# strukturag/libheif

Measured on NVIDIA H100. Metric: megapixels/sec HEIC-grid decode->RGB, higher is better.
Workload: dtype u8

## Files before the change

libheif_b200/csrc/b200_hevc_recon.cu:

```cuda
#include "b200_hevc.h"

namespace b200 {

#ifndef B200_RECON_MIN_BLOCKS
#define B200_RECON_MIN_BLOCKS 5
#endif
constexpr int WARPS = 4;
constexpr int PAD = 16;
constexpr int MT32_OFF = 0, MT16_OFF = 32 * 36, MT8_OFF = MT16_OFF + 16 * 20;
constexpr int MAT_BYTES = MT8_OFF + 8 * 12;
constexpr int REF_STRIDE = 136;

struct WarpLayout { int tile, top, res, tmp, desc, total; };
__host__ __device__ inline WarpLayout warp_layout(int log2ctb, int bps) {
  const int ctb = 1 << log2ctb, tb = ctb < 32 ? ctb : 32;
  WarpLayout L; int o = 0;
  L.tile = o; o += ctb * (ctb + PAD) * bps;
  L.top = o; o += (2 * PAD + 2 * ctb + 32) * bps;
  o = (o + 15) & ~15;
  L.res = o; o += ctb * ctb * 2;
  L.tmp = o; o += (tb * (tb + 2) * 2 > 1024 ? tb * (tb + 2) * 2 : 1024);
  L.desc = o; o += (ctb / 4) * (ctb / 4) * 8;
  L.total = (o + 15) & ~15;
  return L;
}

__constant__ int8_t c_dct[32] = {64, 90, 90, 90, 89, 88, 87, 85, 83, 82, 80, 78, 75, 73, 70, 67,
                                 64, 61, 57, 54, 50, 46, 43, 38, 36, 31, 25, 22, 18, 13, 9, 4};
__constant__ int8_t c_angle[35] = {0, 0, 32, 26, 21, 17, 13, 9, 5, 2, 0, -2, -5, -9, -13, -17, -21, -26, -32,
                                   -26, -21, -17, -13, -9, -5, -2, 0, 2, 5, 9, 13, 17, 21, 26, 32};
__constant__ int16_t c_inv_angle[35] = {0, 0, 0, 0, 0, 0, 0, 0, 0, 0, 0, -4096, -1638, -910, -630, -482, -390, -315, -256,
                                        -315, -390, -482, -630, -910, -1638, -4096, 0, 0, 0, 0, 0, 0, 0, 0, 0};
__constant__ uint8_t c_qpc[14] = {29, 30, 31, 32, 33, 33, 34, 34, 35, 35, 36, 36, 37, 37};
__constant__ uint8_t c_level_scale[6] = {40, 45, 51, 57, 64, 72};

__device__ __forceinline__ int clip3i(int lo, int hi, int v) { return min(max(v, lo), hi); }
__device__ __forceinline__ unsigned morton4(unsigned x, unsigned y) {
  unsigned sx = (x & 1) | ((x & 2) << 1) | ((x & 4) << 2) | ((x & 8) << 3);
  unsigned sy = (y & 1) | ((y & 2) << 1) | ((y & 4) << 2) | ((y & 8) << 3);
  return sx | (sy << 1);
}
__device__ __forceinline__ unsigned ld_acquire(const unsigned* p) {
  unsigned v; asm volatile("ld.relaxed.gpu.global.u32 %0, [%1];" : "=r"(v) : "l"(p) : "memory"); return v;
}
__device__ __forceinline__ void st_release(unsigned* p, unsigned v) {
  asm volatile("st.release.gpu.global.u32 [%0], %1;" ::"l"(p), "r"(v) : "memory");
}
__device__ __forceinline__ void bulk_store(void* g, const void* s, unsigned bytes) {
  asm volatile("cp.async.bulk.global.shared::cta.bulk_group [%0], [%1], %2;" ::"l"(g), "r"((unsigned)__cvta_generic_to_shared(s)), "r"(bytes) : "memory");
}

template <bool LIVE, class T> __device__ __forceinline__ T ld_cmd(const T* p) { return LIVE ? __ldcg(p) : *p; }
template <bool LIVE> __device__ __forceinline__ TuCmd ld_tu(const TuCmd* p) { const uint4 v = ld_cmd<LIVE>(reinterpret_cast<const uint4*>(p)); return TuCmd{v.x, v.y, v.z, v.w}; }
template <bool LIVE> __device__ __forceinline__ CoefEntry ld_coef(const CoefEntry* p) { const unsigned v = ld_cmd<LIVE>(reinterpret_cast<const unsigned*>(p)); CoefEntry e; e.pos = (uint16_t)(v & 0xffff); e.level = (int16_t)(v >> 16); return e; }
template <bool LIVE> __device__ __forceinline__ CtuInfo ld_ctu(const CtuInfo* p) {
  CtuInfo c; const uint2* s = reinterpret_cast<const uint2*>(p); uint2* d = reinterpret_cast<uint2*>(&c);
#pragma unroll
  for (int i = 0; i < (int)(sizeof(CtuInfo) / 8); i++) d[i] = ld_cmd<LIVE>(s + i);
  return c;
}

__device__ __forceinline__ int chroma_qp(int qpy, int off, int bd, int cfmt = 1) {
  const int qbd = 6 * (bd - 8);
  const int qpi = clip3i(-qbd, 57, qpy + off);
  const int qpc = cfmt != 1 ? min(qpi, 51) : (qpi < 30 ? qpi : (qpi >= 43 ? qpi - 6 : c_qpc[qpi - 30]));
  return qpc + qbd;
}

__device__ __forceinline__ int dequant(int level, int qp, int bd_shift, int m) {
  const long long scale = (long long)(c_level_scale[qp % 6] << (qp / 6)) * m;
  const long long t = ((long long)level * scale + (1LL << (bd_shift - 1))) >> bd_shift;
  return (int)(t < -32768 ? -32768 : (t > 32767 ? 32767 : t));
}

__device__ __forceinline__ unsigned make_desc(int bx, int by, int lg, int mode, int coded0, int coded1, int tw, int th, int shx, int cx0, int cy0, int cw, int ch,
                                              bool nbL, bool nbAL, bool nbA, bool nbAR) {
  const int n = 1 << lg;
  const bool fL = bx > 0 || nbL, fT = by > 0 || nbA;
  const bool fC = (bx > 0 && by > 0) ? true : (bx > 0 ? nbA : (by > 0 ? nbL : nbAL));
  const unsigned me = morton4((unsigned)(bx << shx) >> 2, (unsigned)by >> 2);
  bool tr = false, bl = false;
  if (cx0 + bx + n < cw) {
    if (by > 0) { if (bx + n < tw) tr = morton4((unsigned)((bx + n) << shx) >> 2, (unsigned)(by - 1) >> 2) < me; }
    else tr = (bx + n < tw) ? nbA : nbAR;
  }
  if (cy0 + by + n < ch && by + n < th) {
    if (bx > 0) bl = morton4((unsigned)((bx - 1) << shx) >> 2, (unsigned)(by + n) >> 2) < me; else bl = nbL;
  }
  const int trc = tr ? min(n, cw - (cx0 + bx + n)) : 0, blc = bl ? min(n, ch - (cy0 + by + n)) : 0;
  return (unsigned)(bx >> 2) | ((unsigned)(by >> 2) << 4) | ((unsigned)(lg - 2) << 8) | ((unsigned)mode << 10) | ((unsigned)coded0 << 16) | ((unsigned)coded1 << 17) |
         ((unsigned)fL << 18) | ((unsigned)fC << 19) | ((unsigned)fT << 20) | ((unsigned)(blc >> 2) << 21) | ((unsigned)(trc >> 2) << 25);
}

template <bool LIVE>
__device__ __forceinline__ void residual4_lane(int16_t* scr, int lane, const CoefEntry* __restrict__ ce, int nnz, int qp, int bd, bool dst, bool tskip, bool raw, int16_t* out,
                                               const uint8_t* __restrict__ sf) {
  int16_t* my = scr + lane;
#pragma unroll
  for (int p = 0; p < 16; p++) my[p * 32] = 0;
  const int bd_shift = bd - 3;
#pragma unroll 1
  for (int i = 0; i < nnz; i++) {
    const CoefEntry e = ld_coef<LIVE>(&ce[i]);
    my[(e.pos & 15) * 32] = raw ? e.level : (int16_t)dequant(e.level, qp, bd_shift, sf ? (int)__ldg(sf + (e.pos & 15)) : 16);
  }
  int c[16];
#pragma unroll
  for (int p = 0; p < 16; p++) c[p] = my[p * 32];
  const int bs2 = 20 - bd, rnd = 1 << (bs2 - 1);
  unsigned* o32 = reinterpret_cast<unsigned*>(out);
  if (raw) {
#pragma unroll
    for (int p = 0; p < 16; p += 2) o32[p >> 1] = (unsigned)(c[p] & 0xffff) | ((unsigned)c[p + 1] << 16);
    return;
  }
  if (tskip) {
#pragma unroll
    for (int p = 0; p < 16; p += 2) {
      const int r0 = ((c[p] << 7) + rnd) >> bs2, r1 = ((c[p + 1] << 7) + rnd) >> bs2;
      o32[p >> 1] = (unsigned)(r0 & 0xffff) | ((unsigned)r1 << 16);
    }
    return;
  }
  int t[16];
#pragma unroll
  for (int x = 0; x < 4; x++) {
    const int c0 = c[x], c1 = c[4 + x], c2 = c[8 + x], c3 = c[12 + x];
    int e0, e1, e2, e3;
    if (dst) {
      e0 = 29 * c0 + 74 * c1 + 84 * c2 + 55 * c3; e1 = 55 * c0 + 74 * c1 - 29 * c2 - 84 * c3;
      e2 = 74 * c0 - 74 * c2 + 74 * c3;           e3 = 84 * c0 - 74 * c1 + 55 * c2 - 29 * c3;
    } else {
      const int a = 64 * (c0 + c2), b = 64 * (c0 - c2), o0 = 83 * c1 + 36 * c3, o1 = 36 * c1 - 83 * c3;
      e0 = a + o0; e1 = b + o1; e2 = b - o1; e3 = a - o0;
    }
    t[x * 4 + 0] = clip3i(-32768, 32767, (e0 + 64) >> 7); t[x * 4 + 1] = clip3i(-32768, 32767, (e1 + 64) >> 7);
    t[x * 4 + 2] = clip3i(-32768, 32767, (e2 + 64) >> 7); t[x * 4 + 3] = clip3i(-32768, 32767, (e3 + 64) >> 7);
  }
#pragma unroll
  for (int y = 0; y < 4; y++) {
    const int c0 = t[y], c1 = t[4 + y], c2 = t[8 + y], c3 = t[12 + y];
    int e0, e1, e2, e3;
    if (dst) {
      e0 = 29 * c0 + 74 * c1 + 84 * c2 + 55 * c3; e1 = 55 * c0 + 74 * c1 - 29 * c2 - 84 * c3;
      e2 = 74 * c0 - 74 * c2 + 74 * c3;           e3 = 84 * c0 - 74 * c1 + 55 * c2 - 29 * c3;
    } else {
      const int a = 64 * (c0 + c2), b = 64 * (c0 - c2), o0 = 83 * c1 + 36 * c3, o1 = 36 * c1 - 83 * c3;
      e0 = a + o0; e1 = b + o1; e2 = b - o1; e3 = a - o0;
    }
    const int r0 = (e0 + rnd) >> bs2, r1 = (e1 + rnd) >> bs2, r2 = (e2 + rnd) >> bs2, r3 = (e3 + rnd) >> bs2;
    o32[y * 2] = (unsigned)(r0 & 0xffff) | ((unsigned)r1 << 16);
    o32[y * 2 + 1] = (unsigned)(r2 & 0xffff) | ((unsigned)r3 << 16);
  }
}

template <bool LIVE>
__device__ __noinline__ void residual_big(int16_t* rs, int16_t* tmp, const int8_t* __restrict__ mat, const CoefEntry* __restrict__ ce, int nnz, int lg, int qp, int bd, int lane,
                                          const uint8_t* __restrict__ sf, int sf_dc, bool raw) {
  const int n = 1 << lg;
  unsigned* z = reinterpret_cast<unsigned*>(rs);
#pragma unroll 1
  for (int i = lane; i < n * n / 2; i += 32) z[i] = 0;
  __syncwarp();
  const int bd_shift = bd + lg - 5;
  int maxrow = 0, maxcol = 0;
#pragma unroll 1
  for (int i = lane; i < nnz; i += 32) {
    const CoefEntry e = ld_coef<LIVE>(&ce[i]);
    const int pos = e.pos & (n * n - 1);
    const int x = pos & (n - 1), y = pos >> lg;
    int m = 16;
    if (sf) m = (pos == 0 && lg >= 4) ? sf_dc : (int)__ldg(sf + ((y >> (lg - 3)) << 3) + (x >> (lg - 3)));
    rs[raw ? pos : x * n + y] = raw ? e.level : (int16_t)dequant(e.level, qp, bd_shift, m);
    maxrow = max(maxrow, y); maxcol = max(maxcol, x);
  }
  maxrow = __reduce_max_sync(0xffffffffu, maxrow); maxcol = __reduce_max_sync(0xffffffffu, maxcol);
  __syncwarp();
  if (raw) return;
  const int8_t* mt = mat + (lg == 5 ? MT32_OFF : (lg == 4 ? MT16_OFF : MT8_OFF));
  const int ms = n + 4, P2 = n + 2;
  const int kq1 = (maxrow >> 2) + 1, ncol = ((maxcol >> 2) + 1) << 2;
#pragma unroll 1
  for (int i = lane; i < n * ncol; i += 32) {
    const int y = i & (n - 1), x = i >> lg;
    const int2* c = reinterpret_cast<const int2*>(rs + x * n);
    const int* mq = reinterpret_cast<const int*>(mt + y * ms);
    int e = 0;
#pragma unroll 2
    for (int q = 0; q < kq1; q++) { const int2 a = c[q]; const int bq = mq[q]; e = __dp2a_lo(a.x, bq, e); e = __dp2a_hi(a.y, bq, e); }
    tmp[y * P2 + x] = (int16_t)clip3i(-32768, 32767, (e + 64) >> 7);
  }
  __syncwarp();
  const int bs2 = 20 - bd, rnd = 1 << (bs2 - 1), kq2 = ncol >> 2;
#pragma unroll 1
  for (int p = lane; p < n * n; p += 32) {
    const int x = p & (n - 1), y = p >> lg;
    const int* u = reinterpret_cast<const int*>(tmp + y * P2);
    const int* mq = reinterpret_cast<const int*>(mt + x * ms);
    int e = 0;
#pragma unroll 2
    for (int q = 0; q < kq2; q++) { const int bq = mq[q]; e = __dp2a_lo(u[2 * q], bq, e); e = __dp2a_hi(u[2 * q + 1], bq, e); }
    rs[p] = (int16_t)((e + rnd) >> bs2);
  }
  __syncwarp();
}

template <typename P>
__device__ __forceinline__ void predict_tb(const uint2 d, P* tl, const P* tp, const int16_t* rs, int16_t* rf, int S, int l, int lpc, unsigned gmask, int cidx, bool luma, bool smooth, int bd, int strong_en) {
  const int bx = (int)(d.x & 15) << 2, by = (int)((d.x >> 4) & 15) << 2, lg = 2 + (int)((d.x >> 8) & 3), mode = (int)((d.x >> 10) & 63);
  const int n = 1 << lg, n2 = 2 * n, n4 = 4 * n;
  const bool coded = (d.x >> (16 + cidx)) & 1, pcm = (d.x >> 29) & 1;
  const bool fL = (d.x >> 18) & 1, fC = (d.x >> 19) & 1, fT = (d.x >> 20) & 1;
  const int blc = (int)((d.x >> 21) & 15) << 2, trc = (int)((d.x >> 25) & 15) << 2;
  const int first = blc ? n - blc : (fL ? n : (fC ? n2 : (fT ? n2 + 1 : (trc ? 3 * n + 1 : -1))));
  const P* colL = tl + by * S + PAD + bx - 1;
  const P* rowA = (by > 0 ? tl + (by - 1) * S : tp) + PAD + bx;
  int dcs = 0;
  const bool small = n4 < lpc;
  const int jn = small ? n4 + 1 : n4;
#pragma unroll 1
  for (int j = l; j < jn; j += lpc) {
    const int i = j == n4 ? n2 : (j < n2 ? j : j + 1);
    int v = 1 << (bd - 1);
    if (first >= 0) {
      int s = first;
      if (blc && i >= n - blc) s = min(i, n - 1);
      if (fL && i >= n) s = min(i, n2 - 1);
      if (fC && i >= n2) s = n2;
      if (fT && i > n2) s = min(i, 3 * n);
      if (trc && i > 3 * n) s = min(i, 3 * n + trc);
      v = s < n2 ? (int)colL[(n2 - 1 - s) * S] : (int)rowA[s - n2 - 1];
    }
    rf[i] = (int16_t)v;
    if ((i >= n && i < n2) || (i > n2 && i <= 3 * n)) dcs += v;
  }
  if (!small && l == 0) {
    int v = 1 << (bd - 1);
    if (first >= 0) {
      int s = first;
      if (blc) s = n - 1;
      if (fL) s = n2 - 1;
      if (fC) s = n2;
      v = s < n2 ? (int)colL[(n2 - 1 - s) * S] : (int)rowA[s - n2 - 1];
    }
    rf[n2] = (int16_t)v;
  }
  __syncwarp();
  const int16_t* ref = rf;
  if (smooth && mode != 1 && n != 4) {
    const int dist = min(abs(mode - 26), abs(mode - 10));
    const int thr = n == 8 ? 7 : (n == 16 ? 1 : 0);
    if (dist > thr) {
      const int corner = rf[n2], bl = rf[0], tr = rf[n4];
      const bool strong = strong_en && n == 32 && abs(corner + tr - 2 * rf[3 * n]) < (1 << (bd - 5)) && abs(corner + bl - 2 * rf[n]) < (1 << (bd - 5));
      int16_t* rb = rf + REF_STRIDE;
#pragma unroll 1
      for (int i = l; i <= n4; i += lpc) {
        int v;
        if (i == 0 || i == n4) v = rf[i];
        else if (strong) {
          if (i == n2) v = corner;
          else if (i < n2) { const int y = n2 - 1 - i; v = ((63 - y) * corner + (y + 1) * bl + 32) >> 6; }
          else { const int x = i - n2 - 1; v = ((63 - x) * corner + (x + 1) * tr + 32) >> 6; }
        } else v = (rf[i - 1] + 2 * rf[i] + rf[i + 1] + 2) >> 2;
        rb[i] = (int16_t)v;
      }
      __syncwarp();
      ref = rb;
    }
  }
  const int maxv = (1 << bd) - 1;
#define LEFT(y) ((int)ref[n2 - 1 - (y)])
#define TOP(x) ((int)ref[n2 + 1 + (x)])
  int dc = 0;
  if (mode == 1) dc = (__reduce_add_sync(gmask, dcs) + n) >> (lg + 1);
  const int ang = c_angle[mode], ia = c_inv_angle[mode];
  const bool edge = luma && n < 32;
  const int16_t* rsb = rs + d.y;
  P* out = tl + by * S + PAD + bx;
#pragma unroll 1
  for (int e = l; e < n * n; e += lpc) {
    const int x = e & (n - 1), y = e >> lg;
    int v;
    if (pcm) { out[y * S + x] = (P)rsb[e]; continue; }
    if (mode == 0) v = ((n - 1 - x) * LEFT(y) + (x + 1) * TOP(n) + (n - 1 - y) * TOP(x) + (y + 1) * LEFT(n) + n) >> (lg + 1);
    else if (mode == 1) {
      v = dc;
      if (edge) {
        if (x == 0 && y == 0) v = (LEFT(0) + 2 * dc + TOP(0) + 2) >> 2;
        else if (y == 0) v = (TOP(x) + 3 * dc + 2) >> 2;
        else if (x == 0) v = (LEFT(y) + 3 * dc + 2) >> 2;
      }
    } else if (mode >= 18) {
      const int idx = ((y + 1) * ang) >> 5, f = ((y + 1) * ang) & 31;
      const int k0 = x + idx + 1, k1 = k0 + 1;
      const int a = k0 >= 0 ? TOP(k0 - 1) : LEFT(-1 + ((k0 * ia + 128) >> 8));
      if (f) { const int b = k1 >= 0 ? TOP(k1 - 1) : LEFT(-1 + ((k1 * ia + 128) >> 8)); v = ((32 - f) * a + f * b + 16) >> 5; } else v = a;
      if (mode == 26 && edge && x == 0) v = clip3i(0, maxv, TOP(0) + ((LEFT(y) - LEFT(-1)) >> 1));
    } else {
      const int idx = ((x + 1) * ang) >> 5, f = ((x + 1) * ang) & 31;
      const int k0 = y + idx + 1, k1 = k0 + 1;
      const int a = k0 >= 0 ? LEFT(k0 - 1) : TOP(-1 + ((k0 * ia + 128) >> 8));
      if (f) { const int b = k1 >= 0 ? LEFT(k1 - 1) : TOP(-1 + ((k1 * ia + 128) >> 8)); v = ((32 - f) * a + f * b + 16) >> 5; } else v = a;
      if (mode == 10 && edge && y == 0) v = clip3i(0, maxv, LEFT(0) + ((TOP(x) - TOP(-1)) >> 1));
    }
    if (coded) v = clip3i(0, maxv, v + (int)rsb[e]);
    out[y * S + x] = (P)v;
  }
#undef LEFT
#undef TOP
  __syncwarp();
}

template <typename P, bool LIVE>
__global__ void __launch_bounds__(WARPS * 32, B200_RECON_MIN_BLOCKS) hevc_recon_kernel(const DeviceBatch b) {
  extern __shared__ __align__(16) unsigned char smem_raw[];
  int8_t* mat = reinterpret_cast<int8_t*>(smem_raw);
  for (int i = threadIdx.x; i < 1024 + 256 + 64; i += blockDim.x) {
    const int lg = i < 1024 ? 5 : (i < 1280 ? 4 : 3), j0 = i < 1024 ? i : (i < 1280 ? i - 1024 : i - 1280);
    const int n = 1 << lg, y = j0 >> lg, kn = j0 & (n - 1), k = kn << (5 - lg);
    int v;
    if (k == 0) v = 64;
    else { int j = (k * (2 * y + 1)) & 127, sgn = 1; if (j > 64) j = 128 - j; if (j > 32) { j = 64 - j; sgn = -1; } v = sgn * c_dct[j]; }
    mat[(lg == 5 ? MT32_OFF : (lg == 4 ? MT16_OFF : MT8_OFF)) + y * (n + 4) + kn] = (int8_t)v;
  }
  __syncthreads();
  const int lane = threadIdx.x & 31;
  const WarpLayout L = warp_layout(b.max_log2_ctb, (int)sizeof(P));
  unsigned char* wb = smem_raw + MAT_BYTES + (threadIdx.x >> 5) * L.total;
  P* const tile0 = reinterpret_cast<P*>(wb + L.tile);
  P* const top0 = reinterpret_cast<P*>(wb + L.top);
  int16_t* const res0 = reinterpret_cast<int16_t*>(wb + L.res);
  int16_t* const tmp = reinterpret_cast<int16_t*>(wb + L.tmp);
  uint2* const desc = reinterpret_cast<uint2*>(wb + L.desc);
  const unsigned lt_mask = (1u << lane) - 1u;

  for (;;) {
    unsigned t = 0;
    if (lane == 0) t = atomicAdd(b.ticket, 1u);
    t = __shfl_sync(0xffffffffu, t, 0);
    if (t >= (unsigned)b.nrows) break;
    const uint2 pr = b.row_list[t];
    const PicDesc* pic = &b.pics[pr.x];
    const int g = (int)(pr.y >> 30), ry = (int)(pr.y & 0x3fffffffu);
    const int pl = g >= 2 ? g - 1 : 0;
    const int cfmt = pic->chroma;
    const int shx = g == 0 ? 0 : (g == 1 ? 1 : (cfmt == 2 ? 1 : 0)), shy = g == 1 ? 1 : 0;
    const bool paired = g == 1;
    const CtuInfo* ctus = b.ctus + pic->ctu_base;
    const SliceInfo* slices = b.slices + pic->slice_base;
    const int log2ctb = pic->log2_ctb, wctb = pic->wctb, bd = pic->bit_depth, strong_en = pic->strong_intra;
    const int tw = (1 << log2ctb) >> shx, th = (1 << log2ctb) >> shy, S = tw + PAD;
    const int cw = pic->width >> shx, ch = pic->height >> shy;
    const int y0 = ry << log2ctb, cy0 = y0 >> shy;
    const uint8_t* sfac = pic->scaling_idx >= 0 ? b.scaling + (size_t)pic->scaling_idx * 784 : nullptr;
    const TuCmd* tus = b.tus + pic->tu_base;
    const CoefEntry* coefs = b.coefs + pic->coef_base;
    unsigned* prog = b.progress + 3 * pic->progress_base + (g == 3 ? 2 : (g ? 1 : 0));
    const unsigned* eprog = b.entropy_progress ? b.entropy_progress + pic->progress_base : nullptr;
    const int lpc = paired ? 16 : 32, l = lane & (lpc - 1), cidx = paired ? lane >> 4 : 0;
    const unsigned gmask = paired ? (0xffffu << (16 * cidx)) : 0xffffffffu;
    P* const tl = tile0 + cidx * (th * S);
    P* const tp = top0 + cidx * (PAD + 2 * tw + 16);
    int16_t* const rs = res0 + cidx * (tw * th);
    int16_t* const rf = tmp + cidx * REF_STRIDE;
    const int plane = paired ? 1 + cidx : pl;
    P* const recp = static_cast<P*>(pic->rec[plane]);
    const int rst = pic->rec_stride[plane];

    for (int rx = 0; rx < wctb; rx++) {
      const int x0 = rx << log2ctb, cx0 = x0 >> shx;
      if (eprog) {
        int abort = 0;
        if (lane == 0) {
          unsigned spins = 0, ns = 250;
          while (ld_acquire(&eprog[ry]) < (unsigned)(rx + 1)) {
            __nanosleep(ns); if (ns < 8000) ns <<= 1;
            if ((++spins & 31u) == 0 && ld_acquire(b.error_flag)) break;
            if (spins > (1u << 23)) { atomicExch(b.error_flag, 1u); break; }
          }
          abort = ld_acquire(b.error_flag) != 0u;
        }
        if (__shfl_sync(0xffffffffu, abort, 0)) return;
      }
      const int addr = ry * wctb + rx;
      const CtuInfo ci = ld_ctu<LIVE>(&ctus[addr]);
      const int cur = ci.slice_idx;
      const bool nbL = rx > 0 && (int)ld_cmd<LIVE>(&ctus[addr - 1].slice_idx) == cur;
      const bool nbAL = rx > 0 && ry > 0 && (int)ld_cmd<LIVE>(&ctus[addr - wctb - 1].slice_idx) == cur;
      const bool nbA = ry > 0 && (int)ld_cmd<LIVE>(&ctus[addr - wctb].slice_idx) == cur;
      const bool nbAR = ry > 0 && rx + 1 < wctb && (int)ld_cmd<LIVE>(&ctus[addr - wctb + 1].slice_idx) == cur;
      const SliceInfo sl = slices[cur];
      int ntb = 0;
#pragma unroll 1
      for (unsigned base = 0; base < ci.tu_count; base += 32) {
        const bool valid = base + lane < ci.tu_count;
        TuCmd cmd{0, 0, 0, 0};
        if (valid) cmd = ld_tu<LIVE>(&tus[ci.tu_start + base + lane]);
        const int log2n = 2 + (int)((cmd.w0 >> 24) & 3);
        const int lx = (int)((cmd.w0 & 0xfff) << 2) - x0, ly = (int)(((cmd.w0 >> 12) & 0xfff) << 2) - y0;
        const int qpy = (int)((cmd.w1 >> 12) & 0xff) - 64;
        const bool pcm = (cmd.w1 >> 21) & 1, raw = ((cmd.w1 >> 21) & 3) != 0;
        const int nl = (int)(cmd.w3 & 0x7ff), ncb = (int)((cmd.w3 >> 11) & 0x3ff), ncr = (int)((cmd.w3 >> 21) & 0x3ff);
        const CoefEntry* ce = coefs + cmd.w2;
        bool has; int bx, by, lg, mode, coded0, coded1, qp0, qp1 = 0, ts0, ts1 = 0, n0, n1 = 0; const CoefEntry* ce1 = ce;
        if (!paired) {
          has = valid && (int)((cmd.w1 >> 23) & 3) == pl;
          bx = lx >> shx; by = ly; lg = log2n; mode = (int)(cmd.w1 & 63); coded0 = (int)((cmd.w0 >> 26) & 1); coded1 = 0;
          qp0 = pl == 0 ? qpy + 6 * (bd - 8) : chroma_qp(qpy, pl == 1 ? sl.cb_qp_offset : sl.cr_qp_offset, bd, cfmt);
          ts0 = (int)((cmd.w0 >> 30) & 1); n0 = nl;
        } else {
          has = valid && ((cmd.w0 >> 29) & 1);
          if (log2n > 2) { bx = lx >> 1; by = ly >> 1; lg = log2n - 1; } else { bx = (lx - 4) >> 1; by = (ly - 4) >> 1; lg = 2; }
          mode = (int)((cmd.w1 >> 6) & 63); coded0 = (int)((cmd.w0 >> 27) & 1); coded1 = (int)((cmd.w0 >> 28) & 1);
          qp0 = chroma_qp(qpy, sl.cb_qp_offset, bd); qp1 = chroma_qp(qpy, sl.cr_qp_offset, bd);
          ts0 = (int)((cmd.w0 >> 31) & 1); ts1 = (int)((cmd.w1 >> 20) & 1);
          ce = ce + nl; n0 = ncb; ce1 = ce + ncb; n1 = ncr;
        }
        if (!has) { coded0 = coded1 = 0; bx = by = 0; lg = 2; }
        coded0 = coded0 && n0 > 0; coded1 = coded1 && n1 > 0;
        const unsigned hb = __ballot_sync(0xffffffffu, has);
        const int idx = ntb + __popc(hb & lt_mask);
        const unsigned roff = morton4((unsigned)bx >> 2, (unsigned)by >> 2) * 16;
        if (has) desc[idx] = make_uint2(make_desc(bx, by, lg, mode, coded0, coded1, tw, th, paired ? 0 : shx, cx0, cy0, cw, ch, nbL, nbAL, nbA, nbAR) | ((unsigned)pcm << 29), roff);
        ntb += __popc(hb);
        if (lg == 2) {
#pragma unroll 1
          for (int c2 = 0; c2 < 2; c2++)
            if (c2 ? coded1 : coded0)
              residual4_lane<LIVE>(tmp, lane, c2 ? ce1 : ce, c2 ? n1 : n0, c2 ? qp1 : qp0, bd, g == 0, c2 ? ts1 : ts0, raw, res0 + (c2 ? tw * th : 0) + roff,
                                   sfac ? sfac + (paired ? 1 + c2 : pl) * 256 : nullptr);
        }
        __syncwarp();
        unsigned big0 = __ballot_sync(0xffffffffu, lg > 2 && coded0), big1 = __ballot_sync(0xffffffffu, lg > 2 && coded1);
#pragma unroll 1
        for (int c2 = 0; c2 < 2; c2++) {
          unsigned m = c2 ? big1 : big0;
          while (m) {
            const int src = __ffs(m) - 1; m &= m - 1;
            const unsigned long long cp = __shfl_sync(0xffffffffu, (unsigned long long)(c2 ? ce1 : ce), src);
            const int nn = __shfl_sync(0xffffffffu, c2 ? n1 : n0, src), lgg = __shfl_sync(0xffffffffu, lg, src), qq = __shfl_sync(0xffffffffu, c2 ? qp1 : qp0, src);
            const unsigned ro = __shfl_sync(0xffffffffu, roff, src); const bool rw = __shfl_sync(0xffffffffu, (int)raw, src) != 0;
            residual_big<LIVE>(res0 + (c2 ? tw * th : 0) + ro, tmp, mat, reinterpret_cast<const CoefEntry*>(cp), nn, lgg, qq, bd, lane,
                               sfac ? sfac + (paired ? 1 + c2 : pl) * 256 + (lgg - 2) * 64 : nullptr, sfac ? (int)sfac[768 + (paired ? 1 + c2 : pl) * 4 + (lgg - 2)] : 16, rw);
          }
        }
      }
      __syncwarp();
      if (ry > 0) {
        int abort = 0;
        if (lane == 0) {
          const unsigned need = (unsigned)min(rx + 2, wctb);
          unsigned spins = 0, ns = 250;
          while (ld_acquire(&prog[3 * (ry - 1)]) < need) {
            __nanosleep(ns); if (ns < 8000) ns <<= 1;
            if ((++spins & 31u) == 0 && ld_acquire(b.error_flag)) break;
            if (spins > (1u << 23)) { atomicExch(b.error_flag, 1u); break; }
          }
          abort = ld_acquire(b.error_flag) != 0u;
        }
        if (__shfl_sync(0xffffffffu, abort, 0)) return;
        const int cnt = 1 + 2 * tw;
        const P* grow = recp + (size_t)(cy0 - 1) * rst;
#pragma unroll 1
        for (int i = l; i < cnt; i += lpc) {
          const int gx = cx0 - 1 + i;
          int v = 0;
          if (gx >= 0 && gx < cw) v = (int)__ldcg(grow + gx);
          tp[PAD - 1 + i] = (P)v;
        }
      }
      __syncwarp();
#pragma unroll 1
      for (int k = 0; k < ntb; k++) predict_tb<P>(desc[k], tl, tp, rs, rf, S, l, lpc, gmask, cidx, g == 0, g == 0 || (g >= 2 && cfmt == 3), bd, g == 0 ? strong_en : 0);
      {
        const int w = min(tw, cw - cx0), h = min(th, ch - cy0);
        const unsigned rowb = (unsigned)(w * (int)sizeof(P));
        P* gdst = recp + (size_t)cy0 * rst + cx0;
        if ((rowb & 15u) == 0) {
          asm volatile("fence.proxy.async.shared::cta;" ::: "memory");
          __syncwarp();
#pragma unroll 1
          for (int y = l; y < h; y += lpc) bulk_store(gdst + (size_t)y * rst, tl + y * S + PAD, rowb);
          asm volatile("cp.async.bulk.commit_group;" ::: "memory");
        } else {
          const int wq = (int)(rowb >> 2);
#pragma unroll 1
          for (int i = l; i < h * wq; i += lpc) {
            const int y = i / wq, q = i - y * wq;
            reinterpret_cast<unsigned*>(gdst + (size_t)y * rst)[q] = reinterpret_cast<const unsigned*>(tl + y * S + PAD)[q];
          }
        }
        P keep0 = 0, keep1 = 0;
        if (l < th) keep0 = tl[l * S + PAD + tw - 1];
        if (l + lpc < th) keep1 = tl[(l + lpc) * S + PAD + tw - 1];
        if ((rowb & 15u) == 0) asm volatile("cp.async.bulk.wait_group 0;" ::: "memory");
        __syncwarp();
        if (l < th) tl[l * S + PAD - 1] = keep0;
        if (l + lpc < th) tl[(l + lpc) * S + PAD - 1] = keep1;
        __threadfence();
        __syncwarp();
        if (lane == 0) st_release(&prog[3 * ry], (unsigned)(rx + 1));
      }
    }
  }
}

int launch_recon(const DeviceBatch& b, cudaStream_t s) {
  if (b.nrows <= 0) return B200_OK;
  const bool live = b.entropy_progress != nullptr;
  const int bps = b.wide_samples ? 2 : 1;
  const size_t smem = MAT_BYTES + (size_t)warp_layout(b.max_log2_ctb, bps).total * WARPS;
  const void* kern = bps == 2 ? (live ? (const void*)hevc_recon_kernel<uint16_t, true> : (const void*)hevc_recon_kernel<uint16_t, false>)
                              : (live ? (const void*)hevc_recon_kernel<uint8_t, true> : (const void*)hevc_recon_kernel<uint8_t, false>);
  B200_CUDA_CHECK(cudaFuncSetAttribute(kern, cudaFuncAttributeMaxDynamicSharedMemorySize, (int)(MAT_BYTES + (size_t)warp_layout(6, 2).total * WARPS)));
  int dev = 0, sms = 148;
  cudaGetDevice(&dev);
  cudaDeviceGetAttribute(&sms, cudaDevAttrMultiProcessorCount, dev);
  int occ = 1;
  cudaOccupancyMaxActiveBlocksPerMultiprocessor(&occ, kern, WARPS * 32, smem);
  if (occ < 1) occ = 1;
  if (b.blocks_per_sm > 0 && b.blocks_per_sm < occ) occ = b.blocks_per_sm;
  const int want = (b.nrows + WARPS - 1) / WARPS;
  const int grid = want < sms * occ ? want : sms * occ;
  void* args[] = {const_cast<DeviceBatch*>(&b)};
  cudaError_t e = cudaLaunchKernel(kern, dim3((unsigned)grid), dim3(WARPS * 32), args, smem, s);
  if (e != cudaSuccess) return set_error(B200_E_CUDA, "recon launch: %s", cudaGetErrorString(e));
  return B200_OK;
}

}
```

Measured before the change: 4079.

## Cut recon register pressure and precompute intra filter info per descriptor

Moves per-picture pointers (ctus, slices, tus, coefs, progress, recon planes) into a per-warp shared struct so they stop occupying registers. Coefficient offsets become 32-bit. Reference-filter selection and first-available-sample index are computed once when each descriptor is built instead of inside predict_tb. Tu and coef loads no longer use __ldcg in live mode. Residual4 reads coefficients straight from shared scratch instead of a 16-entry register array. The top-row fetch becomes word-wide, the descriptor loop prefetches the next entry, and an optional clock-based trace is added behind a macro. The aim is lower register use and less per-block ALU work, in exchange for extra shared-memory loads through a volatile struct and possible stale reads in live mode now that the cache-bypassing loads are gone.

```diff
diff --git a/libheif_b200/csrc/b200_hevc_recon.cu b/libheif_b200/csrc/b200_hevc_recon.cu
--- a/libheif_b200/csrc/b200_hevc_recon.cu
+++ b/libheif_b200/csrc/b200_hevc_recon.cu
@@ -25,6 +25,8 @@
   return L;
 }
 
+struct ItemPtrs { const CtuInfo* ctus; const SliceInfo* slices; const TuCmd* tus; const CoefEntry* coefs; const uint8_t* sfac; unsigned* prog; const unsigned* eprog; void* recp[2]; };
+
 __constant__ int8_t c_dct[32] = {64, 90, 90, 90, 89, 88, 87, 85, 83, 82, 80, 78, 75, 73, 70, 67,
                                  64, 61, 57, 54, 50, 46, 43, 38, 36, 31, 25, 22, 18, 13, 9, 4};
 __constant__ int8_t c_angle[35] = {0, 0, 32, 26, 21, 17, 13, 9, 5, 2, 0, -2, -5, -9, -13, -17, -21, -26, -32,
@@ -34,6 +36,34 @@
 __constant__ uint8_t c_qpc[14] = {29, 30, 31, 32, 33, 33, 34, 34, 35, 35, 36, 36, 37, 37};
 __constant__ uint8_t c_level_scale[6] = {40, 45, 51, 57, 64, 72};
 
+#ifdef B200_RECON_TRACE
+enum {
+  RT_OTHER, RT_WAIT_K0, RT_A_DESC, RT_A4, RT_ABIG, RT_WAIT_ROW, RT_B4, RT_B8, RT_B16, RT_B32, RT_STORE,
+  RT_CTBS, RT_N4, RT_N8, RT_N16, RT_N32, RT_PLANAR, RT_DC, RT_ANG_V, RT_ANG_H, RT_PCM, RT_SLOTS
+};
+constexpr int RTRACE_WARPS = 4096;
+__device__ unsigned long long g_rtrace[RTRACE_WARPS][RT_SLOTS];
+#define RT_DECL                                                                                     \
+  __shared__ unsigned s_rt[WARPS][RT_SLOTS];                                                        \
+  unsigned* const rt_w = s_rt[threadIdx.x >> 5];                                                    \
+  for (int i = lane; i < RT_SLOTS; i += 32) rt_w[i] = 0;                                            \
+  __syncwarp();                                                                                     \
+  unsigned rt_t = (unsigned)clock()
+#define RT_LAP(s) do { if (lane == 0) { const unsigned rt_now = (unsigned)clock(); rt_w[s] += rt_now - rt_t; rt_t = rt_now; } } while (0)
+#define RT_ADD(s, v) do { if (lane == 0) rt_w[s] += (unsigned)(v); } while (0)
+#define RT_FLUSH                                                                                    \
+  do {                                                                                              \
+    __syncwarp();                                                                                   \
+    const unsigned rt_g = min(blockIdx.x * WARPS + (threadIdx.x >> 5), RTRACE_WARPS - 1u);         \
+    for (int i = lane; i < RT_SLOTS; i += 32) atomicAdd(&g_rtrace[rt_g][i], (unsigned long long)rt_w[i]); \
+  } while (0)
+#else
+#define RT_DECL do {} while (0)
+#define RT_LAP(s) do {} while (0)
+#define RT_ADD(s, v) do {} while (0)
+#define RT_FLUSH do {} while (0)
+#endif
+
 __device__ __forceinline__ int clip3i(int lo, int hi, int v) { return min(max(v, lo), hi); }
 __device__ __forceinline__ unsigned morton4(unsigned x, unsigned y) {
   unsigned sx = (x & 1) | ((x & 2) << 1) | ((x & 4) << 2) | ((x & 8) << 3);
@@ -51,8 +81,8 @@
 }
 
 template <bool LIVE, class T> __device__ __forceinline__ T ld_cmd(const T* p) { return LIVE ? __ldcg(p) : *p; }
-template <bool LIVE> __device__ __forceinline__ TuCmd ld_tu(const TuCmd* p) { const uint4 v = ld_cmd<LIVE>(reinterpret_cast<const uint4*>(p)); return TuCmd{v.x, v.y, v.z, v.w}; }
-template <bool LIVE> __device__ __forceinline__ CoefEntry ld_coef(const CoefEntry* p) { const unsigned v = ld_cmd<LIVE>(reinterpret_cast<const unsigned*>(p)); CoefEntry e; e.pos = (uint16_t)(v & 0xffff); e.level = (int16_t)(v >> 16); return e; }
+__device__ __forceinline__ TuCmd ld_tu(const TuCmd* p) { const uint4 v = *reinterpret_cast<const uint4*>(p); return TuCmd{v.x, v.y, v.z, v.w}; }
+__device__ __forceinline__ CoefEntry ld_coef(const CoefEntry* p) { const unsigned v = *reinterpret_cast<const unsigned*>(p); CoefEntry e; e.pos = (uint16_t)(v & 0xffff); e.level = (int16_t)(v >> 16); return e; }
 template <bool LIVE> __device__ __forceinline__ CtuInfo ld_ctu(const CtuInfo* p) {
   CtuInfo c; const uint2* s = reinterpret_cast<const uint2*>(p); uint2* d = reinterpret_cast<uint2*>(&c);
 #pragma unroll
@@ -73,26 +103,34 @@
   return (int)(t < -32768 ? -32768 : (t > 32767 ? 32767 : t));
 }
 
-__device__ __forceinline__ unsigned make_desc(int bx, int by, int lg, int mode, int coded0, int coded1, int tw, int th, int shx, int cx0, int cy0, int cw, int ch,
-                                              bool nbL, bool nbAL, bool nbA, bool nbAR) {
+__device__ __forceinline__ uint2 make_desc(int bx, int by, int lg, int mode, int coded0, int coded1, bool pcm, unsigned roff, int tw, int th, int shx, int rw, int rh,
+                                           unsigned nb, bool smooth, bool strong_en) {
   const int n = 1 << lg;
+  const bool nbL = nb & 1, nbAL = nb & 2, nbA = nb & 4, nbAR = nb & 8;
   const bool fL = bx > 0 || nbL, fT = by > 0 || nbA;
   const bool fC = (bx > 0 && by > 0) ? true : (bx > 0 ? nbA : (by > 0 ? nbL : nbAL));
   const unsigned me = morton4((unsigned)(bx << shx) >> 2, (unsigned)by >> 2);
   bool tr = false, bl = false;
-  if (cx0 + bx + n < cw) {
+  if (bx + n < rw) {
     if (by > 0) { if (bx + n < tw) tr = morton4((unsigned)((bx + n) << shx) >> 2, (unsigned)(by - 1) >> 2) < me; }
     else tr = (bx + n < tw) ? nbA : nbAR;
   }
-  if (cy0 + by + n < ch && by + n < th) {
+  if (by + n < rh && by + n < th) {
     if (bx > 0) bl = morton4((unsigned)((bx - 1) << shx) >> 2, (unsigned)(by + n) >> 2) < me; else bl = nbL;
   }
-  const int trc = tr ? min(n, cw - (cx0 + bx + n)) : 0, blc = bl ? min(n, ch - (cy0 + by + n)) : 0;
-  return (unsigned)(bx >> 2) | ((unsigned)(by >> 2) << 4) | ((unsigned)(lg - 2) << 8) | ((unsigned)mode << 10) | ((unsigned)coded0 << 16) | ((unsigned)coded1 << 17) |
-         ((unsigned)fL << 18) | ((unsigned)fC << 19) | ((unsigned)fT << 20) | ((unsigned)(blc >> 2) << 21) | ((unsigned)(trc >> 2) << 25);
-}
-
-template <bool LIVE>
+  const int trc = tr ? min(n, rw - (bx + n)) : 0, blc = bl ? min(n, rh - (by + n)) : 0;
+  const int n2 = 2 * n, first = blc ? n - blc : (fL ? n : (fC ? n2 : (fT ? n2 + 1 : (trc ? 3 * n + 1 : -1))));
+  unsigned filt = 0;
+  if (smooth && mode != 1 && n != 4) {
+    const int dist = min(abs(mode - 26), abs(mode - 10));
+    if (dist > (n == 8 ? 7 : (n == 16 ? 1 : 0))) filt = strong_en && n == 32 ? 2 : 1;
+  }
+  return make_uint2((unsigned)(bx >> 2) | ((unsigned)(by >> 2) << 4) | ((unsigned)(lg - 2) << 8) | ((unsigned)mode << 10) | ((unsigned)coded0 << 16) |
+                        ((unsigned)coded1 << 17) | ((unsigned)fL << 18) | ((unsigned)fC << 19) | ((unsigned)fT << 20) | ((unsigned)(blc >> 2) << 21) |
+                        ((unsigned)(trc >> 2) << 25) | ((unsigned)pcm << 29),
+                    roff | ((unsigned)(first + 1) << 12) | (filt << 20));
+}
+
 __device__ __forceinline__ void residual4_lane(int16_t* scr, int lane, const CoefEntry* __restrict__ ce, int nnz, int qp, int bd, bool dst, bool tskip, bool raw, int16_t* out,
                                                const uint8_t* __restrict__ sf) {
   int16_t* my = scr + lane;
@@ -101,23 +139,20 @@
   const int bd_shift = bd - 3;
 #pragma unroll 1
   for (int i = 0; i < nnz; i++) {
-    const CoefEntry e = ld_coef<LIVE>(&ce[i]);
+    const CoefEntry e = ld_coef(&ce[i]);
     my[(e.pos & 15) * 32] = raw ? e.level : (int16_t)dequant(e.level, qp, bd_shift, sf ? (int)__ldg(sf + (e.pos & 15)) : 16);
   }
-  int c[16];
-#pragma unroll
-  for (int p = 0; p < 16; p++) c[p] = my[p * 32];
   const int bs2 = 20 - bd, rnd = 1 << (bs2 - 1);
   unsigned* o32 = reinterpret_cast<unsigned*>(out);
   if (raw) {
 #pragma unroll
-    for (int p = 0; p < 16; p += 2) o32[p >> 1] = (unsigned)(c[p] & 0xffff) | ((unsigned)c[p + 1] << 16);
+    for (int p = 0; p < 16; p += 2) o32[p >> 1] = (unsigned)(my[p * 32] & 0xffff) | ((unsigned)my[(p + 1) * 32] << 16);
     return;
   }
   if (tskip) {
 #pragma unroll
     for (int p = 0; p < 16; p += 2) {
-      const int r0 = ((c[p] << 7) + rnd) >> bs2, r1 = ((c[p + 1] << 7) + rnd) >> bs2;
+      const int r0 = (((int)my[p * 32] << 7) + rnd) >> bs2, r1 = (((int)my[(p + 1) * 32] << 7) + rnd) >> bs2;
       o32[p >> 1] = (unsigned)(r0 & 0xffff) | ((unsigned)r1 << 16);
     }
     return;
@@ -125,7 +160,7 @@
   int t[16];
 #pragma unroll
   for (int x = 0; x < 4; x++) {
-    const int c0 = c[x], c1 = c[4 + x], c2 = c[8 + x], c3 = c[12 + x];
+    const int c0 = my[x * 32], c1 = my[(4 + x) * 32], c2 = my[(8 + x) * 32], c3 = my[(12 + x) * 32];
     int e0, e1, e2, e3;
     if (dst) {
       e0 = 29 * c0 + 74 * c1 + 84 * c2 + 55 * c3; e1 = 55 * c0 + 74 * c1 - 29 * c2 - 84 * c3;
@@ -154,7 +189,6 @@
   }
 }
 
-template <bool LIVE>
 __device__ __noinline__ void residual_big(int16_t* rs, int16_t* tmp, const int8_t* __restrict__ mat, const CoefEntry* __restrict__ ce, int nnz, int lg, int qp, int bd, int lane,
                                           const uint8_t* __restrict__ sf, int sf_dc, bool raw) {
   const int n = 1 << lg;
@@ -166,7 +200,7 @@
   int maxrow = 0, maxcol = 0;
 #pragma unroll 1
   for (int i = lane; i < nnz; i += 32) {
-    const CoefEntry e = ld_coef<LIVE>(&ce[i]);
+    const CoefEntry e = ld_coef(&ce[i]);
     const int pos = e.pos & (n * n - 1);
     const int x = pos & (n - 1), y = pos >> lg;
     int m = 16;
@@ -206,13 +240,13 @@
 }
 
 template <typename P>
-__device__ __forceinline__ void predict_tb(const uint2 d, P* tl, const P* tp, const int16_t* rs, int16_t* rf, int S, int l, int lpc, unsigned gmask, int cidx, bool luma, bool smooth, int bd, int strong_en) {
+__device__ __forceinline__ void predict_tb(const uint2 d, P* tl, const P* tp, const int16_t* rs, int16_t* rf, int S, int l, int lpc, unsigned gmask, int cidx, bool luma, int bd) {
   const int bx = (int)(d.x & 15) << 2, by = (int)((d.x >> 4) & 15) << 2, lg = 2 + (int)((d.x >> 8) & 3), mode = (int)((d.x >> 10) & 63);
   const int n = 1 << lg, n2 = 2 * n, n4 = 4 * n;
   const bool coded = (d.x >> (16 + cidx)) & 1, pcm = (d.x >> 29) & 1;
   const bool fL = (d.x >> 18) & 1, fC = (d.x >> 19) & 1, fT = (d.x >> 20) & 1;
   const int blc = (int)((d.x >> 21) & 15) << 2, trc = (int)((d.x >> 25) & 15) << 2;
-  const int first = blc ? n - blc : (fL ? n : (fC ? n2 : (fT ? n2 + 1 : (trc ? 3 * n + 1 : -1))));
+  const int first = (int)((d.y >> 12) & 255) - 1;
   const P* colL = tl + by * S + PAD + bx - 1;
   const P* rowA = (by > 0 ? tl + (by - 1) * S : tp) + PAD + bx;
   int dcs = 0;
@@ -247,27 +281,24 @@
   }
   __syncwarp();
   const int16_t* ref = rf;
-  if (smooth && mode != 1 && n != 4) {
-    const int dist = min(abs(mode - 26), abs(mode - 10));
-    const int thr = n == 8 ? 7 : (n == 16 ? 1 : 0);
-    if (dist > thr) {
-      const int corner = rf[n2], bl = rf[0], tr = rf[n4];
-      const bool strong = strong_en && n == 32 && abs(corner + tr - 2 * rf[3 * n]) < (1 << (bd - 5)) && abs(corner + bl - 2 * rf[n]) < (1 << (bd - 5));
-      int16_t* rb = rf + REF_STRIDE;
-#pragma unroll 1
-      for (int i = l; i <= n4; i += lpc) {
-        int v;
-        if (i == 0 || i == n4) v = rf[i];
-        else if (strong) {
-          if (i == n2) v = corner;
-          else if (i < n2) { const int y = n2 - 1 - i; v = ((63 - y) * corner + (y + 1) * bl + 32) >> 6; }
-          else { const int x = i - n2 - 1; v = ((63 - x) * corner + (x + 1) * tr + 32) >> 6; }
-        } else v = (rf[i - 1] + 2 * rf[i] + rf[i + 1] + 2) >> 2;
-        rb[i] = (int16_t)v;
-      }
-      __syncwarp();
-      ref = rb;
-    }
+  const unsigned filt = (d.y >> 20) & 3;
+  if (filt) {
+    const int corner = rf[n2], bl = rf[0], tr = rf[n4];
+    const bool strong = filt == 2 && abs(corner + tr - 2 * rf[3 * n]) < (1 << (bd - 5)) && abs(corner + bl - 2 * rf[n]) < (1 << (bd - 5));
+    int16_t* rb = rf + REF_STRIDE;
+#pragma unroll 1
+    for (int i = l; i <= n4; i += lpc) {
+      int v;
+      if (i == 0 || i == n4) v = rf[i];
+      else if (strong) {
+        if (i == n2) v = corner;
+        else if (i < n2) { const int y = n2 - 1 - i; v = ((63 - y) * corner + (y + 1) * bl + 32) >> 6; }
+        else { const int x = i - n2 - 1; v = ((63 - x) * corner + (x + 1) * tr + 32) >> 6; }
+      } else v = (rf[i - 1] + 2 * rf[i] + rf[i + 1] + 2) >> 2;
+      rb[i] = (int16_t)v;
+    }
+    __syncwarp();
+    ref = rb;
   }
   const int maxv = (1 << bd) - 1;
 #define LEFT(y) ((int)ref[n2 - 1 - (y)])
@@ -276,7 +307,7 @@
   if (mode == 1) dc = (__reduce_add_sync(gmask, dcs) + n) >> (lg + 1);
   const int ang = c_angle[mode], ia = c_inv_angle[mode];
   const bool edge = luma && n < 32;
-  const int16_t* rsb = rs + d.y;
+  const int16_t* rsb = rs + (d.y & 0xfff);
   P* out = tl + by * S + PAD + bx;
 #pragma unroll 1
   for (int e = l; e < n * n; e += lpc) {
@@ -334,6 +365,9 @@
   int16_t* const tmp = reinterpret_cast<int16_t*>(wb + L.tmp);
   uint2* const desc = reinterpret_cast<uint2*>(wb + L.desc);
   const unsigned lt_mask = (1u << lane) - 1u;
+  __shared__ ItemPtrs s_items[WARPS];
+  volatile ItemPtrs& it = s_items[threadIdx.x >> 5];
+  RT_DECL;
 
   for (;;) {
     unsigned t = 0;
@@ -347,17 +381,20 @@
     const int cfmt = pic->chroma;
     const int shx = g == 0 ? 0 : (g == 1 ? 1 : (cfmt == 2 ? 1 : 0)), shy = g == 1 ? 1 : 0;
     const bool paired = g == 1;
-    const CtuInfo* ctus = b.ctus + pic->ctu_base;
-    const SliceInfo* slices = b.slices + pic->slice_base;
-    const int log2ctb = pic->log2_ctb, wctb = pic->wctb, bd = pic->bit_depth, strong_en = pic->strong_intra;
+    const int log2ctb = pic->log2_ctb, wctb = pic->wctb, bd = pic->bit_depth;
+    const bool smooth = g == 0 || (g >= 2 && cfmt == 3), strong_en = g == 0 && pic->strong_intra;
     const int tw = (1 << log2ctb) >> shx, th = (1 << log2ctb) >> shy, S = tw + PAD;
     const int cw = pic->width >> shx, ch = pic->height >> shy;
     const int y0 = ry << log2ctb, cy0 = y0 >> shy;
-    const uint8_t* sfac = pic->scaling_idx >= 0 ? b.scaling + (size_t)pic->scaling_idx * 784 : nullptr;
-    const TuCmd* tus = b.tus + pic->tu_base;
-    const CoefEntry* coefs = b.coefs + pic->coef_base;
-    unsigned* prog = b.progress + 3 * pic->progress_base + (g == 3 ? 2 : (g ? 1 : 0));
-    const unsigned* eprog = b.entropy_progress ? b.entropy_progress + pic->progress_base : nullptr;
+    if (lane == 0) {
+      it.ctus = b.ctus + pic->ctu_base;
+      it.slices = b.slices + pic->slice_base;
+      it.sfac = pic->scaling_idx >= 0 ? b.scaling + (size_t)pic->scaling_idx * 784 : nullptr;
+      it.tus = b.tus + pic->tu_base;
+      it.coefs = b.coefs + pic->coef_base;
+      it.prog = b.progress + 3 * pic->progress_base + (g == 3 ? 2 : (g ? 1 : 0));
+      it.eprog = b.entropy_progress ? b.entropy_progress + pic->progress_base : nullptr;
+    }
     const int lpc = paired ? 16 : 32, l = lane & (lpc - 1), cidx = paired ? lane >> 4 : 0;
     const unsigned gmask = paired ? (0xffffu << (16 * cidx)) : 0xffffffffu;
     P* const tl = tile0 + cidx * (th * S);
@@ -365,12 +402,15 @@
     int16_t* const rs = res0 + cidx * (tw * th);
     int16_t* const rf = tmp + cidx * REF_STRIDE;
     const int plane = paired ? 1 + cidx : pl;
-    P* const recp = static_cast<P*>(pic->rec[plane]);
+    if (lane == 0 || lane == 16) it.recp[cidx] = pic->rec[plane];
     const int rst = pic->rec_stride[plane];
+    __syncwarp();
 
     for (int rx = 0; rx < wctb; rx++) {
       const int x0 = rx << log2ctb, cx0 = x0 >> shx;
-      if (eprog) {
+      RT_LAP(RT_OTHER);
+      RT_ADD(RT_CTBS, 1);
+      if (const unsigned* eprog = it.eprog) {
         int abort = 0;
         if (lane == 0) {
           unsigned spins = 0, ns = 250;
@@ -383,27 +423,29 @@
         }
         if (__shfl_sync(0xffffffffu, abort, 0)) return;
       }
+      RT_LAP(RT_WAIT_K0);
       const int addr = ry * wctb + rx;
+      const CtuInfo* ctus = it.ctus;
       const CtuInfo ci = ld_ctu<LIVE>(&ctus[addr]);
       const int cur = ci.slice_idx;
-      const bool nbL = rx > 0 && (int)ld_cmd<LIVE>(&ctus[addr - 1].slice_idx) == cur;
-      const bool nbAL = rx > 0 && ry > 0 && (int)ld_cmd<LIVE>(&ctus[addr - wctb - 1].slice_idx) == cur;
-      const bool nbA = ry > 0 && (int)ld_cmd<LIVE>(&ctus[addr - wctb].slice_idx) == cur;
-      const bool nbAR = ry > 0 && rx + 1 < wctb && (int)ld_cmd<LIVE>(&ctus[addr - wctb + 1].slice_idx) == cur;
-      const SliceInfo sl = slices[cur];
+      const unsigned nb = (unsigned)(rx > 0 && (int)ld_cmd<LIVE>(&ctus[addr - 1].slice_idx) == cur) |
+                          ((unsigned)(rx > 0 && ry > 0 && (int)ld_cmd<LIVE>(&ctus[addr - wctb - 1].slice_idx) == cur) << 1) |
+                          ((unsigned)(ry > 0 && (int)ld_cmd<LIVE>(&ctus[addr - wctb].slice_idx) == cur) << 2) |
+                          ((unsigned)(ry > 0 && rx + 1 < wctb && (int)ld_cmd<LIVE>(&ctus[addr - wctb + 1].slice_idx) == cur) << 3);
+      const SliceInfo sl = it.slices[cur];
       int ntb = 0;
 #pragma unroll 1
       for (unsigned base = 0; base < ci.tu_count; base += 32) {
         const bool valid = base + lane < ci.tu_count;
         TuCmd cmd{0, 0, 0, 0};
-        if (valid) cmd = ld_tu<LIVE>(&tus[ci.tu_start + base + lane]);
+        if (valid) cmd = ld_tu(&it.tus[ci.tu_start + base + lane]);
         const int log2n = 2 + (int)((cmd.w0 >> 24) & 3);
         const int lx = (int)((cmd.w0 & 0xfff) << 2) - x0, ly = (int)(((cmd.w0 >> 12) & 0xfff) << 2) - y0;
         const int qpy = (int)((cmd.w1 >> 12) & 0xff) - 64;
         const bool pcm = (cmd.w1 >> 21) & 1, raw = ((cmd.w1 >> 21) & 3) != 0;
         const int nl = (int)(cmd.w3 & 0x7ff), ncb = (int)((cmd.w3 >> 11) & 0x3ff), ncr = (int)((cmd.w3 >> 21) & 0x3ff);
-        const CoefEntry* ce = coefs + cmd.w2;
-        bool has; int bx, by, lg, mode, coded0, coded1, qp0, qp1 = 0, ts0, ts1 = 0, n0, n1 = 0; const CoefEntry* ce1 = ce;
+        unsigned ce = cmd.w2;
+        bool has; int bx, by, lg, mode, coded0, coded1, qp0, qp1 = 0, ts0, ts1 = 0, n0, n1 = 0; unsigned ce1 = ce;
         if (!paired) {
           has = valid && (int)((cmd.w1 >> 23) & 3) == pl;
           bx = lx >> shx; by = ly; lg = log2n; mode = (int)(cmd.w1 & 63); coded0 = (int)((cmd.w0 >> 26) & 1); coded1 = 0;
@@ -415,42 +457,47 @@
           mode = (int)((cmd.w1 >> 6) & 63); coded0 = (int)((cmd.w0 >> 27) & 1); coded1 = (int)((cmd.w0 >> 28) & 1);
           qp0 = chroma_qp(qpy, sl.cb_qp_offset, bd); qp1 = chroma_qp(qpy, sl.cr_qp_offset, bd);
           ts0 = (int)((cmd.w0 >> 31) & 1); ts1 = (int)((cmd.w1 >> 20) & 1);
-          ce = ce + nl; n0 = ncb; ce1 = ce + ncb; n1 = ncr;
+          ce += nl; n0 = ncb; ce1 = ce + ncb; n1 = ncr;
         }
         if (!has) { coded0 = coded1 = 0; bx = by = 0; lg = 2; }
         coded0 = coded0 && n0 > 0; coded1 = coded1 && n1 > 0;
         const unsigned hb = __ballot_sync(0xffffffffu, has);
         const int idx = ntb + __popc(hb & lt_mask);
         const unsigned roff = morton4((unsigned)bx >> 2, (unsigned)by >> 2) * 16;
-        if (has) desc[idx] = make_uint2(make_desc(bx, by, lg, mode, coded0, coded1, tw, th, paired ? 0 : shx, cx0, cy0, cw, ch, nbL, nbAL, nbA, nbAR) | ((unsigned)pcm << 29), roff);
+        if (has) desc[idx] = make_desc(bx, by, lg, mode, coded0, coded1, pcm, roff, tw, th, paired ? 0 : shx, cw - cx0, ch - cy0, nb, smooth, strong_en);
         ntb += __popc(hb);
+        RT_LAP(RT_A_DESC);
+        const uint8_t* const sfac = it.sfac;
         if (lg == 2) {
 #pragma unroll 1
           for (int c2 = 0; c2 < 2; c2++)
             if (c2 ? coded1 : coded0)
-              residual4_lane<LIVE>(tmp, lane, c2 ? ce1 : ce, c2 ? n1 : n0, c2 ? qp1 : qp0, bd, g == 0, c2 ? ts1 : ts0, raw, res0 + (c2 ? tw * th : 0) + roff,
+              residual4_lane(tmp, lane, it.coefs + (c2 ? ce1 : ce), c2 ? n1 : n0, c2 ? qp1 : qp0, bd, g == 0, c2 ? ts1 : ts0, raw, res0 + (c2 ? tw * th : 0) + roff,
                                    sfac ? sfac + (paired ? 1 + c2 : pl) * 256 : nullptr);
         }
         __syncwarp();
+        RT_LAP(RT_A4);
         unsigned big0 = __ballot_sync(0xffffffffu, lg > 2 && coded0), big1 = __ballot_sync(0xffffffffu, lg > 2 && coded1);
 #pragma unroll 1
         for (int c2 = 0; c2 < 2; c2++) {
           unsigned m = c2 ? big1 : big0;
           while (m) {
             const int src = __ffs(m) - 1; m &= m - 1;
-            const unsigned long long cp = __shfl_sync(0xffffffffu, (unsigned long long)(c2 ? ce1 : ce), src);
+            const unsigned cp = __shfl_sync(0xffffffffu, c2 ? ce1 : ce, src);
             const int nn = __shfl_sync(0xffffffffu, c2 ? n1 : n0, src), lgg = __shfl_sync(0xffffffffu, lg, src), qq = __shfl_sync(0xffffffffu, c2 ? qp1 : qp0, src);
             const unsigned ro = __shfl_sync(0xffffffffu, roff, src); const bool rw = __shfl_sync(0xffffffffu, (int)raw, src) != 0;
-            residual_big<LIVE>(res0 + (c2 ? tw * th : 0) + ro, tmp, mat, reinterpret_cast<const CoefEntry*>(cp), nn, lgg, qq, bd, lane,
+            residual_big(res0 + (c2 ? tw * th : 0) + ro, tmp, mat, it.coefs + cp, nn, lgg, qq, bd, lane,
                                sfac ? sfac + (paired ? 1 + c2 : pl) * 256 + (lgg - 2) * 64 : nullptr, sfac ? (int)sfac[768 + (paired ? 1 + c2 : pl) * 4 + (lgg - 2)] : 16, rw);
           }
         }
+        RT_LAP(RT_ABIG);
       }
       __syncwarp();
       if (ry > 0) {
         int abort = 0;
         if (lane == 0) {
           const unsigned need = (unsigned)min(rx + 2, wctb);
+          const unsigned* prog = it.prog;
           unsigned spins = 0, ns = 250;
           while (ld_acquire(&prog[3 * (ry - 1)]) < need) {
             __nanosleep(ns); if (ns < 8000) ns <<= 1;
@@ -460,23 +507,36 @@
           abort = ld_acquire(b.error_flag) != 0u;
         }
         if (__shfl_sync(0xffffffffu, abort, 0)) return;
-        const int cnt = 1 + 2 * tw;
-        const P* grow = recp + (size_t)(cy0 - 1) * rst;
-#pragma unroll 1
-        for (int i = l; i < cnt; i += lpc) {
-          const int gx = cx0 - 1 + i;
-          int v = 0;
-          if (gx >= 0 && gx < cw) v = (int)__ldcg(grow + gx);
-          tp[PAD - 1 + i] = (P)v;
+        const int spw = 4 / (int)sizeof(P), nw = 2 * tw / spw;
+        const P* grow = static_cast<const P*>(it.recp[cidx]) + (size_t)(cy0 - 1) * rst;
+#pragma unroll 1
+        for (int q = l; q <= nw; q += lpc) {
+          if (q == nw) tp[PAD - 1] = cx0 > 0 ? __ldcg(grow + cx0 - 1) : (P)0;
+          else {
+            const int gx = cx0 + q * spw;
+            reinterpret_cast<unsigned*>(tp + PAD)[q] = gx < cw ? __ldcg(reinterpret_cast<const unsigned*>(grow + gx)) : 0u;
+          }
         }
       }
       __syncwarp();
-#pragma unroll 1
-      for (int k = 0; k < ntb; k++) predict_tb<P>(desc[k], tl, tp, rs, rf, S, l, lpc, gmask, cidx, g == 0, g == 0 || (g >= 2 && cfmt == 3), bd, g == 0 ? strong_en : 0);
+      RT_LAP(RT_WAIT_ROW);
+      uint2 dn = desc[0];
+#pragma unroll 1
+      for (int k = 0; k < ntb; k++) {
+        const uint2 dk = dn;
+        if (k + 1 < ntb) dn = desc[k + 1];
+        predict_tb<P>(dk, tl, tp, rs, rf, S, l, lpc, gmask, cidx, g == 0, bd);
+#ifdef B200_RECON_TRACE
+        const unsigned dx = dk.x, lgi = (dx >> 8) & 3, md = (dx >> 10) & 63;
+        RT_LAP(RT_B4 + lgi);
+        RT_ADD(RT_N4 + lgi, 1);
+        RT_ADD((dx >> 29) & 1 ? RT_PCM : (md == 0 ? RT_PLANAR : (md == 1 ? RT_DC : (md >= 18 ? RT_ANG_V : RT_ANG_H))), 1);
+#endif
+      }
       {
         const int w = min(tw, cw - cx0), h = min(th, ch - cy0);
         const unsigned rowb = (unsigned)(w * (int)sizeof(P));
-        P* gdst = recp + (size_t)cy0 * rst + cx0;
+        P* gdst = static_cast<P*>(it.recp[cidx]) + (size_t)cy0 * rst + cx0;
         if ((rowb & 15u) == 0) {
           asm volatile("fence.proxy.async.shared::cta;" ::: "memory");
           __syncwarp();
@@ -500,11 +560,29 @@
         if (l + lpc < th) tl[(l + lpc) * S + PAD - 1] = keep1;
         __threadfence();
         __syncwarp();
-        if (lane == 0) st_release(&prog[3 * ry], (unsigned)(rx + 1));
+        if (lane == 0) st_release(&it.prog[3 * ry], (unsigned)(rx + 1));
       }
-    }
-  }
-}
+      RT_LAP(RT_STORE);
+    }
+  }
+  RT_FLUSH;
+}
+
+#ifdef B200_RECON_TRACE
+extern "C" int b200_debug_recon_trace(unsigned long long* out, int nwarps) {
+  if (!out || nwarps < 0 || nwarps > RTRACE_WARPS) return set_error(B200_E_INVALID, "bad trace request");
+  static unsigned long long t[RTRACE_WARPS][RT_SLOTS];
+  cudaError_t e = cudaDeviceSynchronize();
+  if (e == cudaSuccess) e = cudaMemcpyFromSymbol(t, g_rtrace, sizeof t);
+  if (e == cudaSuccess) {
+    memcpy(out, t, sizeof t[0] * nwarps);
+    memset(t, 0, sizeof t);
+    e = cudaMemcpyToSymbol(g_rtrace, t, sizeof t);
+  }
+  if (e != cudaSuccess) return set_error(B200_E_CUDA, "recon trace: %s", cudaGetErrorString(e));
+  return B200_OK;
+}
+#endif
 
 int launch_recon(const DeviceBatch& b, cudaStream_t s) {
   if (b.nrows <= 0) return B200_OK;
```

Result: faster. 4188 (median of 6 runs) (+2.7%).
